# Onr/Council-GAN

Hardware: NVIDIA H100
Metric: training images/sec (gen+dis step) (higher is better)
Workload: dtype tf32

## Files before the change

council_gan_b200/csrc/api.cu:

```cuda
#include "common.cuh"
#include <string.h>

namespace cg {

static thread_local char g_err[512] = "";
std::atomic<uint64_t> g_launches{0};
thread_local int g_tc_mode = 7;
thread_local int g_pdl = 0;

void set_error(const char* fmt, ...) {
    va_list ap;
    va_start(ap, fmt);
    vsnprintf(g_err, sizeof(g_err), fmt, ap);
    va_end(ap);
}

int validate_geom(const cg_conv_geom& g) {
    CG_REQUIRE(g.G >= 1 && (g.x_groups == 1 || g.x_groups == g.G), "conv: x_groups=%d must be 1 or G=%d", g.x_groups, g.G);
    CG_REQUIRE(g.Cin % 4 == 0 && g.Cin > 0, "conv: Cin=%d must be a positive multiple of 4", g.Cin);
    CG_REQUIRE(g.Cout > 0 && g.B > 0 && g.H > 0 && g.W > 0, "conv: empty tensor");
    CG_REQUIRE(g.stride >= 1 && g.KH >= 1 && g.KW >= 1 && g.pad >= 0, "conv: bad kernel geometry");
    int Hin = g.ups ? 2 * g.H : g.H, Win = g.ups ? 2 * g.W : g.W;
    int Ho = (Hin + 2 * g.pad - g.KH) / g.stride + 1, Wo = (Win + 2 * g.pad - g.KW) / g.stride + 1;
    CG_REQUIRE(Ho == g.Ho && Wo == g.Wo, "conv: output size %dx%d inconsistent with geometry (expected %dx%d)", g.Ho, g.Wo, Ho, Wo);
// ... 91 lines not shown
    }
    if (sm_count) *sm_count = prop.multiProcessorCount;
    if (cc_major) *cc_major = prop.major;
    if (cc_minor) *cc_minor = prop.minor;
    return prop.multiProcessorCount;
}

extern "C" int cg_set_tensor_core_mode(int mode) {
    int prev = g_tc_mode;
    g_tc_mode = mode == 1 ? 7 : (mode & 7);
    g_small_bn = ((mode >> 23) & 1) ? 0 : 1;
    g_wgrad_tma = ((mode >> 25) & 1) ? 0 : 1;
    g_pdl = (mode >> 22) & 1;
    g_tc_serial_epilogue = (mode >> 26) & 1;
    g_tc_reg_epilogue = (mode >> 27) & 1;
    return prev;
}

extern "C" uint64_t cg_launch_count(void) { return g_launches.load(); }
extern "C" void cg_tensor_map_cache_stats(uint64_t* hits, uint64_t* misses) { tc_map_cache_stats(hits, misses); }

extern "C" int cg_zero(void* ptr, size_t bytes, void* stream) {
    cudaError_t e = cudaMemsetAsync(ptr, 0, bytes, (cudaStream_t)stream);
    if (e != cudaSuccess) {
        set_error("cg_zero: %s", cudaGetErrorString(e));
        return CG_ERR_CUDA;
    }
    return CG_OK;
}

// ... 146 lines not shown
```

council_gan_b200/csrc/common.cuh:

```cuda
#pragma once
#include <cuda.h>
#include <cuda_runtime.h>
#include <stdint.h>
#include <stdio.h>
#include <stdarg.h>
#include <atomic>
#include "../../include/council_b200.h"

namespace cg {

void set_error(const char* fmt, ...);
extern std::atomic<uint64_t> g_launches;
extern thread_local int g_tc_mode;
extern thread_local int g_small_bn;
extern thread_local int g_wgrad_tma;
extern thread_local int g_tc_serial_epilogue;
extern thread_local int g_tc_reg_epilogue;

constexpr int CG_MAX_DEVICES = 64;
inline int current_device() {
    int dev = 0;
    cudaGetDevice(&dev);
    return dev >= 0 && dev < CG_MAX_DEVICES ? dev : 0;
}
struct PerDeviceOnce {
    std::atomic<bool> done[CG_MAX_DEVICES];
    bool first() { return !done[current_device()].exchange(true); }
    void reset() { done[current_device()].store(false); }
};

inline int check_launch(const char* what) {
    g_launches.fetch_add(1, std::memory_order_relaxed);
// ... 101 lines not shown
```

council_gan_b200/csrc/conv_tc.cu:

```cuda
#include "common.cuh"
#include "tc_ptx.cuh"
#include <cstdlib>
#include <cstdio>
#include <cuda.h>
#include <mutex>
#include <string.h>

namespace cg {

typedef CUresult (*EncodeTiledFn)(CUtensorMap*, CUtensorMapDataType, cuuint32_t, void*, const cuuint64_t*, const cuuint64_t*,
                                  const cuuint32_t*, const cuuint32_t*, CUtensorMapInterleave, CUtensorMapSwizzle,
                                  CUtensorMapL2promotion, CUtensorMapFloatOOBfill);
typedef CUresult (*EncodeIm2colFn)(CUtensorMap*, CUtensorMapDataType, cuuint32_t, void*, const cuuint64_t*, const cuuint64_t*,
                                   const int*, const int*, cuuint32_t, cuuint32_t, const cuuint32_t*, CUtensorMapInterleave,
                                   CUtensorMapSwizzle, CUtensorMapL2promotion, CUtensorMapFloatOOBfill);
typedef CUresult (*ReplaceAddressFn)(CUtensorMap*, void*);
static EncodeTiledFn g_encode_tiled = nullptr;
static ReplaceAddressFn g_replace_address = nullptr;
static EncodeIm2colFn g_encode_im2col = nullptr;
static int g_sm_count_dev[CG_MAX_DEVICES] = {0};
static int sm_count_now() {
    int dev = current_device();
    if (!g_sm_count_dev[dev]) cudaDeviceGetAttribute(&g_sm_count_dev[dev], cudaDevAttrMultiProcessorCount, dev);
    return g_sm_count_dev[dev];
}
thread_local int g_small_bn = 1;
thread_local int g_tc_serial_epilogue = 0;
thread_local int g_tc_reg_epilogue = 0;
static int g_driver_version = 0;
static std::once_flag g_once;

struct MapKey {
    const void* ptr;
    int64_t a, b;
    int32_t v[8];
    bool operator==(const MapKey& o) const { return ptr == o.ptr && a == o.a && b == o.b && memcmp(v, o.v, sizeof(v)) == 0; }
};
struct MapSlot {
    MapKey key;
    CUtensorMap map;
    bool used;
};
constexpr int MAP_SLOTS = 8192;
// ... 41 lines not shown
            g_encode_tiled = (EncodeTiledFn)fn;
        fn = nullptr;
        if (cudaGetDriverEntryPoint("cuTensorMapEncodeIm2col", &fn, cudaEnableDefault, &q) == cudaSuccess && q == cudaDriverEntryPointSuccess)
            g_encode_im2col = (EncodeIm2colFn)fn;
        fn = nullptr;
        if (cudaGetDriverEntryPoint("cuTensorMapReplaceAddress", &fn, cudaEnableDefault, &q) == cudaSuccess && q == cudaDriverEntryPointSuccess)
            g_replace_address = (ReplaceAddressFn)fn;
        cudaDriverGetVersion(&g_driver_version);
    });
}

constexpr int TC_BM = 128;
constexpr int TC_BK = 32;
constexpr int TC_THREADS = 384;
constexpr int TC_MAX_STAGES = 12;
constexpr int TC_MAX_CLASSES = 4;

struct TcClass {
    CUtensorMap amap;
    int w0, h0;
    int out_h0, out_w0;
    int wrow_off;
    int pad_;
};
struct TcParams {
    CUtensorMap bmap;
    TcClass cls[TC_MAX_CLASSES];
    int ncls;
    int G, xg_images;
    int B, P, Q;
// ... 2 lines not shown
    int bk;
    int cps;
    int n_store;
    int out_H, out_W, out_sh, out_sw;
    int w_rows_per_group;
    float* y; const float* bias; const float* addend; const float* mask_src;
    float* stats;
    long stats_gbc;
    int act; float slope;
    int stages;
    int serial_epilogue;
    CUtensorMap ymap, addmap, maskmap;
    int epi_slots, epi_slot_bytes;
};

__device__ __forceinline__ void tc_tile(const TcParams& p, int t, int MT, int NT, int& mt, int& nt, int& c, int& g) {
    if (p.serial_epilogue) {
        mt = t % MT;
        int r = t / MT;
        nt = r % NT;
        r /= NT;
        c = r % p.ncls;
        g = r / p.ncls;
        return;
    }
    c = t % p.ncls;
    int r = t / p.ncls;
    mt = r % MT;
    r /= MT;
    nt = r % NT;
    g = r / NT;
}

__device__ __forceinline__ void tc_half_coords(const TcParams& p, int g, int mt, int h, int& q, int& n) {
    const int pq = p.P * p.Q;
    const int m = mt * TC_BM + 64 * h;
    const int img = m / pq, rem = m - img * pq;
    const int pp = rem / p.Q;
    q = rem - pp * p.Q;
    n = (g * p.B + img) * (p.out_H / p.out_sh) + pp;
}

template <int BK, int BN>
__global__ void __launch_bounds__(TC_THREADS, 1) conv_tc_kernel(const __grid_constant__ TcParams p) {
    pdl_trigger();
    extern __shared__ __align__(1024) uint8_t smem_raw[];
    uint8_t* smem = reinterpret_cast<uint8_t*>((reinterpret_cast<uintptr_t>(smem_raw) + 1023) & ~(uintptr_t)1023);
    const int wg = __shfl_sync(0xffffffffu, threadIdx.x >> 7, 0), tid = threadIdx.x & 127;
    constexpr int a_bytes = TC_BM * BK * 4;
    constexpr int b_bytes = ((BN * BK * 4) + 1023) & ~1023;
    const int stage_bytes = p.cps * (a_bytes + b_bytes);
    constexpr int tx_chunk = a_bytes + BN * BK * 4;
    constexpr bool tma_epi = BK == 32 && BN >= 64;
    const int epi_slots = tma_epi ? p.epi_slots : 0;
    uint8_t* epi = smem + (size_t)p.stages * stage_bytes;
    uint64_t* full_bar = reinterpret_cast<uint64_t*>(epi + (size_t)epi_slots * p.epi_slot_bytes);
    uint64_t* empty_bar = full_bar + p.stages;
    uint64_t* efull_bar = empty_bar + p.stages;
    uint64_t* eempty_bar = efull_bar + epi_slots;

    const int MT = (p.B * p.P * p.Q + TC_BM - 1) / TC_BM;
    const int NT = (p.Cout + BN - 1) / BN;
    const int tiles = p.G * p.ncls * NT * MT;
    const int kchunks = (p.Cin + BK - 1) / BK;
    const int kiters = p.KH * p.KW * kchunks;

    if (threadIdx.x == 0) {
// ... 6 lines not shown
        if (epi_slots) {
            prefetch_tmap(&p.ymap);
            if (p.addend) prefetch_tmap(&p.addmap);
            if (p.mask_src) prefetch_tmap(&p.maskmap);
        }
        for (int s = 0; s < epi_slots; s++) {
            mbar_init(&efull_bar[s], 1);
            mbar_init(&eempty_bar[s], 2);
        }
        fence_barrier_init();
    }
    __syncthreads();
    pdl_wait();

    if (wg == 0) {
        if (tid == 0) {
            int stage = 0;
            uint32_t phase = 0;
            for (int t = blockIdx.x; t < tiles; t += gridDim.x) {
                int mt, nt, c, g;
                tc_tile(p, t, MT, NT, mt, nt, c, g);
                const TcClass& cl = p.cls[c];
                long m0 = (long)mt * TC_BM;
                int img = (int)(m0 / (p.P * p.Q));
                int rem = (int)(m0 - (long)img * p.P * p.Q);
                int pp = rem / p.Q, qq = rem - pp * p.Q;
                int n_coord = g * p.xg_images + img;
                int w_coord = cl.w0 + qq * p.stride;
                int h_coord = cl.h0 + pp * p.stride;
                int wrow = g * p.w_rows_per_group + cl.wrow_off + nt * BN;
                int kh = 0, kw = 0, kc = 0;
                for (int k0 = 0; k0 < kiters; k0 += p.cps) {
                    const int n = kiters - k0 < p.cps ? kiters - k0 : p.cps;
                    mbar_wait(&empty_bar[stage], phase ^ 1);
                    uint8_t* sa = smem + (size_t)stage * stage_bytes;
                    uint8_t* sb = sa + p.cps * a_bytes;
                    mbar_expect_tx(&full_bar[stage], (uint32_t)(n * tx_chunk));
                    for (int j = 0; j < n; j++) {
                        tma_load_im2col_4d(&cl.amap, &full_bar[stage], sa + j * a_bytes, kc * BK, w_coord, h_coord, n_coord, (uint16_t)kw,
                                           (uint16_t)kh);
                        tma_load_2d(&p.bmap, &full_bar[stage], sb + j * b_bytes, (kh * p.KW + kw) * p.Cin + kc * BK, wrow);
                        if (++kc == kchunks) { kc = 0; if (++kw == p.KW) { kw = 0; ++kh; } }
                    }
                    if (++stage == p.stages) { stage = 0; phase ^= 1; }
                }
            }
        } else if (tid == 32 && epi_slots) {
            const uint32_t ebytes = (p.addend ? 2 * 8192 : 0) + (p.mask_src ? 2 * 8192 : 0);
            int es = 0;
            uint32_t ephase = 0;
            for (int t = blockIdx.x; t < tiles; t += gridDim.x) {
                int mt, nt, c, g;
                tc_tile(p, t, MT, NT, mt, nt, c, g);
                const TcClass& cl = p.cls[c];
                int q[2], n[2];
                tc_half_coords(p, g, mt, 0, q[0], n[0]);
                tc_half_coords(p, g, mt, 1, q[1], n[1]);
                for (int sl = 0; sl < BN / 32; sl++) {
                    mbar_wait(&eempty_bar[es], ephase ^ 1);
                    if (ebytes) {
                        mbar_expect_tx(&efull_bar[es], ebytes);
                        uint8_t* dst = epi + (size_t)es * p.epi_slot_bytes;
                        const int c0 = nt * BN + 32 * sl;
                        for (int h = 0; h < 2; h++) {
                            if (p.addend) tma_load_5d(&p.addmap, &efull_bar[es], dst + h * 8192, c0, cl.out_w0, q[h], cl.out_h0, n[h]);
                            if (p.mask_src)
                                tma_load_5d(&p.maskmap, &efull_bar[es], dst + (p.addend ? 16384 : 0) + h * 8192, c0, cl.out_w0, q[h],
                                            cl.out_h0, n[h]);
                        }
                    } else {
                        mbar_arrive(&efull_bar[es]);
                    }
                    if (++es == epi_slots) { es = 0; ephase ^= 1; }
                }
            }
        }
        return;
    }

    const int cw = wg - 1;
    const int warp4 = tid >> 5, lane = tid & 31;
    const int row0 = cw * 64 + warp4 * 16 + (lane >> 2);
    const int cq = 2 * (lane & 3);
    const uint64_t desc0 = BK == 32 ? make_kmajor_sw128_desc(0) : make_kmajor_sw32_desc(0);
    float acc[BN / 2];
    int stage = 0;
    uint32_t phase = 0;
    int es = 0;
    uint32_t ephase = 0;
    for (int t = blockIdx.x; t < tiles; t += gridDim.x) {
        int mt, nt, c, g;
        tc_tile(p, t, MT, NT, mt, nt, c, g);
        const TcClass& cl = p.cls[c];
        int prev = -1;
        for (int k0 = 0; k0 < kiters; k0 += p.cps) {
            const int n = kiters - k0 < p.cps ? kiters - k0 : p.cps;
            mbar_wait(&full_bar[stage], phase);
            const uint32_t sa = smem_u32(smem + (size_t)stage * stage_bytes) + cw * (64 * BK * 4);
            const uint32_t sb = smem_u32(smem + (size_t)stage * stage_bytes) + p.cps * a_bytes;
            wgmma_fence();
            for (int j = 0; j < n; j++) {
                const uint64_t adesc = desc0 | (uint64_t)(((sa + j * a_bytes) & 0x3FFFF) >> 4);
                const uint64_t bdesc = desc0 | (uint64_t)(((sb + j * b_bytes) & 0x3FFFF) >> 4);
#pragma unroll
                for (int kk = 0; kk < BK / 8; kk++)
                    wgmma_tf32<BN>(acc, adesc + (uint64_t)(kk * 2), bdesc + (uint64_t)(kk * 2), (k0 | j | kk) != 0 ? 1 : 0);
            }
// ... 142 lines not shown
                const int j = j0 + jj, col = 8 * j + cq;
#pragma unroll
                for (int h = 0; h < 2; h++) {
                    if (col >= p.n_store || !valid[h]) continue;
                    float2 o = make_float2(acc[4 * j + 2 * h] + 0.f, acc[4 * j + 2 * h + 1] + 0.f);
                    if (p.addend) { o.x += av[jj][h].x; o.y += av[jj][h].y; }
                    if (p.mask_src) { o.x *= mv[jj][h].x > 0.f ? 1.f : p.slope; o.y *= mv[jj][h].y > 0.f ? 1.f : p.slope; }
                    *reinterpret_cast<float2*>(p.y + out_off[h] + col) = o;
                }
            }
        }
    }
    if (epi_slots && tid == 0) bulk_wait<0>();
}


static int encode_weights_map_raw(CUtensorMap* map, const float* w, long rows, long ktot, int bn, int bk) {
    cuuint64_t dims[2] = {(cuuint64_t)ktot, (cuuint64_t)rows};
    cuuint64_t strides[1] = {(cuuint64_t)ktot * 4};
    cuuint32_t box[2] = {(cuuint32_t)bk, (cuuint32_t)bn};
    cuuint32_t estr[2] = {1, 1};
    CUresult r = g_encode_tiled(map, CU_TENSOR_MAP_DATA_TYPE_TFLOAT32, 2, (void*)w, dims, strides, box, estr,
                                CU_TENSOR_MAP_INTERLEAVE_NONE, bk == 32 ? CU_TENSOR_MAP_SWIZZLE_128B : CU_TENSOR_MAP_SWIZZLE_32B,
                                CU_TENSOR_MAP_L2_PROMOTION_L2_256B, CU_TENSOR_MAP_FLOAT_OOB_FILL_NONE);
    if (r != CUDA_SUCCESS) {
        set_error("cuTensorMapEncodeTiled(weights rows=%ld ktot=%ld bn=%d) failed: %d", rows, ktot, bn, (int)r);
        return CG_ERR_CUDA;
    }
    return CG_OK;
}

static int encode_weights_map(CUtensorMap* map, const float* w, long rows, long ktot, int bn, int bk = TC_BK) {
    MapKey k{};
    k.ptr = w; k.a = rows; k.b = ktot; k.v[0] = bn; k.v[1] = bk; k.v[7] = 1;
    return cached_map(map, k, [&](CUtensorMap* m) { return encode_weights_map_raw(m, w, rows, ktot, bn, bk); });
}

static int encode_weights_map_p(TcParams& p, const float* w, long rows, long ktot) {
    return encode_weights_map(&p.bmap, w, rows, ktot, p.bn, p.bk);
}

static int encode_act_map_raw(CUtensorMap* map, const float* x, long N, int H, int W, int C, int lo_w, int lo_h, int up_w, int up_h,
                              int stride, int bk) {
    cuuint64_t dims[4] = {(cuuint64_t)C, (cuuint64_t)W, (cuuint64_t)H, (cuuint64_t)N};
    cuuint64_t strides[3] = {(cuuint64_t)C * 4, (cuuint64_t)W * C * 4, (cuuint64_t)H * W * C * 4};
    int lower[2] = {lo_w, lo_h};
    int upper[2] = {up_w, up_h};
    cuuint32_t estr[4] = {1, (cuuint32_t)stride, (cuuint32_t)stride, 1};
    CUresult r = g_encode_im2col(map, CU_TENSOR_MAP_DATA_TYPE_TFLOAT32, 4, (void*)x, dims, strides, lower, upper, bk, TC_BM, estr,
                                 CU_TENSOR_MAP_INTERLEAVE_NONE, bk == 32 ? CU_TENSOR_MAP_SWIZZLE_128B : CU_TENSOR_MAP_SWIZZLE_32B,
                                 CU_TENSOR_MAP_L2_PROMOTION_L2_128B, CU_TENSOR_MAP_FLOAT_OOB_FILL_NONE);
    if (r != CUDA_SUCCESS) {
        set_error("cuTensorMapEncodeIm2col(N=%ld H=%d W=%d C=%d corners %d,%d / %d,%d stride %d) failed: %d", N, H, W, C, lo_w, lo_h,
                  up_w, up_h, stride, (int)r);
// ... 67 lines not shown
    if ((long)g.B * (g.ups ? g.H * g.W : g.Ho * g.Wo) < TC_BM) return false;
    return true;
}

template <int BK>
static void (*tc_kernel_for(int bn))(TcParams) {
    switch (bn) {
        case 16: return conv_tc_kernel<BK, 16>;
        case 64: return conv_tc_kernel<BK, 64>;
        case 128: return conv_tc_kernel<BK, 128>;
        case 256: return conv_tc_kernel<BK, 256>;
    }
    return nullptr;
}

static int launch_tc(TcParams& p, cudaStream_t st) {
    int a_bytes = TC_BM * p.bk * 4, b_bytes = ((p.bn * p.bk * 4) + 1023) & ~1023;
    int chunk_bytes = a_bytes + b_bytes;
    int kiters = p.KH * p.KW * ((p.Cin + p.bk - 1) / p.bk);
    int cps = p.bn <= 64 ? 2 : 1;
    if (p.bk == 8) cps = 8;
    while (cps > 1 && (cps > kiters || cps * chunk_bytes > 64 * 1024)) cps >>= 1;
    p.cps = cps;
    int stage_bytes = cps * chunk_bytes;
    int stages = (226 * 1024 - 1024 - 2 * TC_MAX_STAGES * 8) / stage_bytes;
    if (stages > TC_MAX_STAGES) stages = TC_MAX_STAGES;
    if (stages > 4 && stage_bytes >= 48 * 1024) stages = 4;
    if (p.n_store == 0) p.n_store = p.bn;
    p.serial_epilogue = g_tc_serial_epilogue;
    p.epi_slots = 0;
    const int nops = (p.addend ? 1 : 0) + (p.mask_src ? 1 : 0);
    const bool aligned = ((uintptr_t)p.y | (uintptr_t)p.addend | (uintptr_t)p.mask_src) % 16 == 0;
    if (g_replace_address && !g_tc_reg_epilogue && !p.serial_epilogue && p.bk == TC_BK && p.bn >= 64 && p.n_store == p.bn && (long)p.P * p.Q % TC_BM == 0 &&
        (p.Q % 64 == 0 || 64 % p.Q == 0) && p.out_H % p.out_sh == 0 && p.out_W % p.out_sw == 0 && p.Cout % 4 == 0 && aligned) {
        const int slot_bytes = (nops ? nops : 1) * 16384;
        auto slots_beside = [&](int st) { return (int)((227L * 1024 - 1024 - (long)st * stage_bytes - 2 * st * 8) / (slot_bytes + 16)); };
        while (slots_beside(stages) < 2 && stages > 4) stages--;
        const int e = slots_beside(stages);
        if (e >= 2) {
            p.epi_slots = e < 4 ? e : 4;
            p.epi_slot_bytes = slot_bytes;
            const long ni = (long)p.G * p.B;
            const int qbox = p.Q < 64 ? p.Q : 64;
            if (int rc = encode_out_map(&p.ymap, p.y, ni, p.out_H, p.out_W, p.Cout, p.out_sh, p.out_sw, qbox)) return rc;
            if (p.addend)
                if (int rc = encode_out_map(&p.addmap, p.addend, ni, p.out_H, p.out_W, p.Cout, p.out_sh, p.out_sw, qbox)) return rc;
            if (p.mask_src)
                if (int rc = encode_out_map(&p.maskmap, p.mask_src, ni, p.out_H, p.out_W, p.Cout, p.out_sh, p.out_sw, qbox)) return rc;
        }
    }
    p.stages = stages;
    size_t smem = (size_t)stages * stage_bytes + 1024  + 2 * stages * 8 + (size_t)p.epi_slots * (p.epi_slot_bytes + 16);
    void (*kern)(TcParams) = p.bk == 32 ? tc_kernel_for<32>(p.bn) : tc_kernel_for<8>(p.bn);
    if (!kern) {
        set_error("conv_tc: no kernel for N tile %d / K chunk %d", p.bn, p.bk);
        return CG_ERR_ARG;
    }
    static PerDeviceOnce attr_set;
    if (attr_set.first()) {
        for (int bn : {16, 64, 128, 256}) {
            cudaError_t e = cudaFuncSetAttribute(tc_kernel_for<32>(bn), cudaFuncAttributeMaxDynamicSharedMemorySize, 227 * 1024);
            if (e == cudaSuccess) e = cudaFuncSetAttribute(tc_kernel_for<8>(bn), cudaFuncAttributeMaxDynamicSharedMemorySize, 227 * 1024);
            if (e != cudaSuccess) {
                attr_set.reset();
                set_error("cudaFuncSetAttribute(conv_tc_kernel): %s", cudaGetErrorString(e));
                return CG_ERR_CUDA;
            }
        }
    }
    int MT = cdiv((long)p.B * p.P * p.Q, TC_BM);
    long tiles = (long)p.G * p.ncls * ((p.Cout + p.bn - 1) / p.bn) * MT;
    const long slots = sm_count_now();
    int grid = (int)(tiles < slots ? tiles : slots);
    launch_k(kern, grid, TC_THREADS, smem, st, p);
    return check_launch("conv_tc_kernel");
}


__global__ void ups_weight_transform_kernel(const float* __restrict__ w, float* __restrict__ wc, long total, int Cout, int Cin) {
    pdl_trigger();
    pdl_wait();
    long i = (long)blockIdx.x * blockDim.x + threadIdx.x;
    if (i >= total) return;
    int ci = (int)(i % Cin);
    long t = i / Cin;
    int ss = (int)(t % 2); t /= 2;
    int r = (int)(t % 2); t /= 2;
    int co = (int)(t % Cout); t /= Cout;
    int cls = (int)(t % 4);
    int g = (int)(t / 4);
// ... 30 lines not shown
    p.bk = pick_bk(g.Cin);
    long nimg = (long)(g.x_groups == 1 ? 1 : g.G) * g.B;
    p.G = g.G; p.xg_images = g.x_groups == 1 ? 0 : g.B;
    p.B = g.B; p.Cin = g.Cin; p.Cout = g.Cout;
    p.y = y; p.bias = bias; p.addend = nullptr; p.mask_src = nullptr; p.act = act; p.slope = slope;
    if (g.ups) {
        size_t need = tc_fwd_ws(g);
        if (need > ws_bytes) {
            set_error("conv_fwd(tc, upsample classes): workspace %zu < %zu bytes", ws_bytes, need);
            return CG_ERR_WORKSPACE;
        }
        float* wc = (float*)ws;
        long total = (long)g.G * 4 * g.Cout * 4 * g.Cin;
        launch_k(ups_weight_transform_kernel, cdiv(total, 256), 256, 0, st, w, wc, total, g.Cout, g.Cin);
        if (int rc = check_launch("ups_weight_transform")) return rc;
        if (int rc = encode_weights_map_p(p, wc, (long)g.G * 4 * g.Cout, 4L * g.Cin)) return rc;
        for (int c = 0; c < 4; c++) {
            int a = c >> 1, b = c & 1;
            int lo_h = a == 0 ? -1 : 0, lo_w = b == 0 ? -1 : 0;
            int up_h = a == 0 ? -1 : 0, up_w = b == 0 ? -1 : 0;
            if (int rc = encode_act_map(&p.cls[c].amap, x, nimg, g.H, g.W, g.Cin, lo_w, lo_h, up_w, up_h, 1, p.bk)) return rc;
            p.cls[c].w0 = lo_w; p.cls[c].h0 = lo_h; p.cls[c].out_h0 = a; p.cls[c].out_w0 = b; p.cls[c].wrow_off = c * g.Cout;
        }
        p.ncls = 4;
        p.P = g.H; p.Q = g.W; p.KH = 2; p.KW = 2; p.stride = 1;
        p.out_H = g.Ho; p.out_W = g.Wo; p.out_sh = 2; p.out_sw = 2;
        p.w_rows_per_group = 4 * g.Cout;
        return launch_tc(p, st);
    }
    long ktot = (long)g.KH * g.KW * g.Cin;
    if (int rc = encode_weights_map_p(p, w, (long)g.G * g.Cout, ktot)) return rc;
    if (int rc = encode_act_map(&p.cls[0].amap, x, nimg, g.H, g.W, g.Cin, -g.pad, -g.pad, g.pad - (g.KW - 1), g.pad - (g.KH - 1), g.stride,
                                p.bk))
        return rc;
    p.cls[0].w0 = -g.pad; p.cls[0].h0 = -g.pad; p.cls[0].out_h0 = 0; p.cls[0].out_w0 = 0; p.cls[0].wrow_off = 0;
    p.ncls = 1;
    p.P = g.Ho; p.Q = g.Wo;
    p.KH = g.KH; p.KW = g.KW; p.stride = g.stride;
    p.out_H = g.Ho; p.out_W = g.Wo; p.out_sh = 1; p.out_sw = 1;
    p.w_rows_per_group = g.Cout;
    return launch_tc(p, st);
}

__global__ void __launch_bounds__(256) dgrad_weight_transform_kernel(const float* __restrict__ w, float* __restrict__ wt, int Cout, int Cin,
                                                                     int CinP, int KH, int KW, int s) {
    pdl_trigger();
    pdl_wait();
    __shared__ float tile[32][33];
    const int TH = KH / s, TW = KW / s;
    const int cit = (CinP + 31) / 32;
    const int co0 = (blockIdx.x / cit) * 32, ci0 = (blockIdx.x % cit) * 32;
    int t = blockIdx.y;
    const int ss = t % TW; t /= TW;
    const int r = t % TH; t /= TH;
    const int cls = t;
    const int g = blockIdx.z;
// ... 46 lines not shown
    float* wt = (float*)ws;
    const int CinP = g.Cin <= 16 ? 16 : g.Cin;
    size_t wt_bytes = ((size_t)g.G * g.Cout * g.KH * g.KW * CinP * sizeof(float) + 1023) & ~(size_t)1023;
    float* d_seen = g.ups ? (float*)((uint8_t*)ws + wt_bytes) : dx;
    long total = (long)g.G * g.Cout * g.KH * g.KW * CinP;
    (void)total;
    launch_k(dgrad_weight_transform_kernel, dim3(cdiv(g.Cout, 32) * cdiv(CinP, 32), g.KH * g.KW, g.G), dim3(32, 8), 0, st, w, wt, g.Cout, g.Cin, CinP,
                                                                                                                  g.KH, g.KW, s);
    if (int rc = check_launch("dgrad_weight_transform")) return rc;

    TcParams p{};
    p.bn = pick_bn(g.Cin);
    if (p.bn > 64) p.bn = fill_bn(p.bn, (long)g.B * ((g.ups ? 2 * g.H : g.H) / g.stride) * ((g.ups ? 2 * g.W : g.W) / g.stride), g.G * g.stride * g.stride, g.Cin);
    p.n_store = p.bn == 16 ? g.Cin : p.bn;
    p.bk = pick_bk(g.Cout);
    long ktot = (long)TH * TW * g.Cout;
    if (int rc = encode_weights_map_p(p, wt, (long)g.G * ncls * CinP, ktot)) return rc;
    for (int c = 0; c < ncls; c++) {
        int ph = c / s, pw = c - ph * s;
        int ihf = ((ph - g.pad) % s + s) % s, iwf = ((pw - g.pad) % s + s) % s;
        int padl_h = (TH - 1) - (ihf + g.pad - ph) / s, padl_w = (TW - 1) - (iwf + g.pad - pw) / s;
        int Hc = Hin / s, Wc = Win / s;
        int up_h = Hc - g.Ho - padl_h, up_w = Wc - g.Wo - padl_w;
        if (int rc = encode_act_map(&p.cls[c].amap, dy, (long)g.G * g.B, g.Ho, g.Wo, g.Cout, -padl_w, -padl_h, up_w, up_h, 1, p.bk)) return rc;
        p.cls[c].w0 = -padl_w; p.cls[c].h0 = -padl_h;
        p.cls[c].out_h0 = ihf; p.cls[c].out_w0 = iwf;
        p.cls[c].wrow_off = c * CinP;
    }
    p.ncls = ncls;
    p.G = g.G; p.xg_images = g.B;
    p.B = g.B; p.P = Hin / s; p.Q = Win / s;
    p.Cin = g.Cout; p.Cout = g.Cin; p.KH = TH; p.KW = TW; p.stride = 1;
    p.out_H = Hin; p.out_W = Win; p.out_sh = s; p.out_sw = s;
    p.w_rows_per_group = ncls * CinP;
    p.y = d_seen; p.bias = nullptr;
    p.addend = g.ups ? nullptr : addend; p.mask_src = g.ups ? nullptr : mask_src;
    p.act = CG_ACT_NONE; p.slope = mask_slope;
    if (int rc = launch_tc(p, st)) return rc;
    if (g.ups) return pool2x2_sum(d_seen, dx, addend, mask_src, mask_slope, (long)g.G * g.B, g.H, g.W, g.Cin, st);
    return CG_OK;
}


constexpr int WG_BK = 32;

struct WgParams {
    const float* x; const float* dy; float* out;
    int G, xg_images, B, H, W, Ho, Wo, Cin, Cout, KH, KW, stride, pad;
    long Mpix, chunk;
    int ci_tiles;
};

__device__ __forceinline__ float f4_at(const float4& v, int j) { return j == 0 ? v.x : j == 1 ? v.y : j == 2 ? v.z : v.w; }
// ... 525 lines not shown
```

council_gan_b200/csrc/tc_ptx.cuh:

```cuda
#pragma once
#include <cuda.h>
#include <cuda_runtime.h>
#include <stdint.h>

namespace cg {

__device__ __forceinline__ uint32_t smem_u32(const void* p) { return (uint32_t)__cvta_generic_to_shared(p); }

__device__ __forceinline__ void mbar_init(uint64_t* bar, uint32_t count) {
    asm volatile("mbarrier.init.shared::cta.b64 [%0], %1;" ::"r"(smem_u32(bar)), "r"(count));
}
__device__ __forceinline__ void mbar_expect_tx(uint64_t* bar, uint32_t bytes) {
    asm volatile("mbarrier.arrive.expect_tx.shared::cta.b64 _, [%0], %1;" ::"r"(smem_u32(bar)), "r"(bytes) : "memory");
}
__device__ __forceinline__ void mbar_arrive(uint64_t* bar) {
    asm volatile("mbarrier.arrive.shared::cta.b64 _, [%0];" ::"r"(smem_u32(bar)) : "memory");
}
__device__ __forceinline__ void mbar_wait(uint64_t* bar, uint32_t parity) {
    uint32_t done;
    const uint32_t addr = smem_u32(bar);
    do {
        asm volatile(
            "{\n"
            ".reg .pred p;\n"
// ... 33 lines not shown
        "cp.async.bulk.tensor.5d.shared::cluster.global.mbarrier::complete_tx::bytes [%0], [%1, {%3, %4, %5, %6, %7}], [%2];" ::"r"(smem_u32(dst)),
        "l"(map), "r"(smem_u32(bar)), "r"(c0), "r"(c1), "r"(c2), "r"(c3), "r"(c4)
        : "memory");
}
__device__ __forceinline__ void tma_store_5d(const CUtensorMap* map, const void* src, int c0, int c1, int c2, int c3, int c4) {
    asm volatile("cp.async.bulk.tensor.5d.global.shared::cta.tile.bulk_group [%0, {%2, %3, %4, %5, %6}], [%1];" ::"l"(map),
                 "r"(smem_u32(src)), "r"(c0), "r"(c1), "r"(c2), "r"(c3), "r"(c4)
                 : "memory");
}
__device__ __forceinline__ void bulk_commit() { asm volatile("cp.async.bulk.commit_group;" ::: "memory"); }
template <int N>
__device__ __forceinline__ void bulk_wait_read() { asm volatile("cp.async.bulk.wait_group.read %0;" ::"n"(N) : "memory"); }
template <int N>
__device__ __forceinline__ void bulk_wait() { asm volatile("cp.async.bulk.wait_group %0;" ::"n"(N) : "memory"); }
__device__ __forceinline__ void named_bar_sync(int id, int count) { asm volatile("bar.sync %0, %1;" ::"r"(id), "r"(count) : "memory"); }
__device__ __forceinline__ void prefetch_tmap(const CUtensorMap* map) {
    asm volatile("prefetch.tensormap [%0];" ::"l"(map) : "memory");
}

__device__ __forceinline__ uint64_t make_kmajor_sw128_desc(uint32_t smem_addr) {
    uint64_t d = 0;
    d |= (uint64_t)((smem_addr & 0x3FFFF) >> 4);
    d |= (uint64_t)1 << 16;
    d |= (uint64_t)(1024 >> 4) << 32;
    d |= (uint64_t)1 << 62;
    return d;
}
__device__ __forceinline__ uint64_t make_kmajor_sw32_desc(uint32_t smem_addr) {
    uint64_t d = 0;
    d |= (uint64_t)((smem_addr & 0x3FFFF) >> 4);
// ... 86 lines not shown
```

Before: 47.78.

## Add ping-pong consumer warpgroup conv kernel with register reallocation

Adds a ping-pong variant of the TMA/WGMMA implicit-GEMM conv kernel. The two consumer warpgroups take alternate tiles, and turn-taking mbarriers let one warpgroup's epilogue overlap the other's MMA main loop. The producer warpgroup gives up registers via setmaxnreg so the consumers can grow theirs. The N tile is forced to 128 with an N-inner tile order. The path is used by default when the smem epilogue applies and there are enough tiles; the cost is a narrower tile and extra turn synchronisation.

```diff
diff --git a/council_gan_b200/csrc/api.cu b/council_gan_b200/csrc/api.cu
--- a/council_gan_b200/csrc/api.cu
+++ b/council_gan_b200/csrc/api.cu
@@ -129,6 +129,7 @@
     g_pdl = (mode >> 22) & 1;
     g_tc_serial_epilogue = (mode >> 26) & 1;
     g_tc_reg_epilogue = (mode >> 27) & 1;
+    g_tc_coop = (mode >> 28) & 1;
     return prev;
 }
 
diff --git a/council_gan_b200/csrc/common.cuh b/council_gan_b200/csrc/common.cuh
--- a/council_gan_b200/csrc/common.cuh
+++ b/council_gan_b200/csrc/common.cuh
@@ -16,6 +16,7 @@
 extern thread_local int g_wgrad_tma;
 extern thread_local int g_tc_serial_epilogue;
 extern thread_local int g_tc_reg_epilogue;
+extern thread_local int g_tc_coop;
 
 constexpr int CG_MAX_DEVICES = 64;
 inline int current_device() {
diff --git a/council_gan_b200/csrc/conv_tc.cu b/council_gan_b200/csrc/conv_tc.cu
--- a/council_gan_b200/csrc/conv_tc.cu
+++ b/council_gan_b200/csrc/conv_tc.cu
@@ -27,6 +27,7 @@
 thread_local int g_small_bn = 1;
 thread_local int g_tc_serial_epilogue = 0;
 thread_local int g_tc_reg_epilogue = 0;
+thread_local int g_tc_coop = 0;
 static int g_driver_version = 0;
 static std::once_flag g_once;
 
@@ -98,6 +99,7 @@
 constexpr int TC_BK = 32;
 constexpr int TC_THREADS = 384;
 constexpr int TC_MAX_STAGES = 12;
+constexpr int TC_PP_BN = 128;
 constexpr int TC_MAX_CLASSES = 4;
 
 struct TcClass {
@@ -130,7 +132,17 @@
     int epi_slots, epi_slot_bytes;
 };
 
+template <bool N_INNER>
 __device__ __forceinline__ void tc_tile(const TcParams& p, int t, int MT, int NT, int& mt, int& nt, int& c, int& g) {
+    if constexpr (N_INNER) {
+        c = t % p.ncls;
+        int r = t / p.ncls;
+        nt = r % NT;
+        r /= NT;
+        mt = r % MT;
+        g = r / MT;
+        return;
+    }
     if (p.serial_epilogue) {
         mt = t % MT;
         int r = t / MT;
@@ -155,6 +167,77 @@
     const int pp = rem / p.Q;
     q = rem - pp * p.Q;
     n = (g * p.B + img) * (p.out_H / p.out_sh) + pp;
+}
+
+template <int BK, int BN, bool N_INNER>
+__device__ __forceinline__ void tc_produce(const TcParams& p, uint8_t* smem, uint64_t* full_bar, uint64_t* empty_bar, int tiles, int MT,
+                                           int NT, int kchunks, int kiters, int stage_bytes) {
+    constexpr int a_bytes = TC_BM * BK * 4;
+    constexpr int b_bytes = ((BN * BK * 4) + 1023) & ~1023;
+    constexpr int tx_chunk = a_bytes + BN * BK * 4;
+    int stage = 0;
+    uint32_t phase = 0;
+    for (int t = blockIdx.x; t < tiles; t += gridDim.x) {
+        int mt, nt, c, g;
+        tc_tile<N_INNER>(p, t, MT, NT, mt, nt, c, g);
+        const TcClass& cl = p.cls[c];
+        long m0 = (long)mt * TC_BM;
+        int img = (int)(m0 / (p.P * p.Q));
+        int rem = (int)(m0 - (long)img * p.P * p.Q);
+        int pp = rem / p.Q, qq = rem - pp * p.Q;
+        int n_coord = g * p.xg_images + img;
+        int w_coord = cl.w0 + qq * p.stride;
+        int h_coord = cl.h0 + pp * p.stride;
+        int wrow = g * p.w_rows_per_group + cl.wrow_off + nt * BN;
+        int kh = 0, kw = 0, kc = 0;
+        for (int k0 = 0; k0 < kiters; k0 += p.cps) {
+            const int n = kiters - k0 < p.cps ? kiters - k0 : p.cps;
+            mbar_wait(&empty_bar[stage], phase ^ 1);
+            uint8_t* sa = smem + (size_t)stage * stage_bytes;
+            uint8_t* sb = sa + p.cps * a_bytes;
+            mbar_expect_tx(&full_bar[stage], (uint32_t)(n * tx_chunk));
+            for (int j = 0; j < n; j++) {
+                tma_load_im2col_4d(&cl.amap, &full_bar[stage], sa + j * a_bytes, kc * BK, w_coord, h_coord, n_coord, (uint16_t)kw,
+                                   (uint16_t)kh);
+                tma_load_2d(&p.bmap, &full_bar[stage], sb + j * b_bytes, (kh * p.KW + kw) * p.Cin + kc * BK, wrow);
+                if (++kc == kchunks) { kc = 0; if (++kw == p.KW) { kw = 0; ++kh; } }
+            }
+            if (++stage == p.stages) { stage = 0; phase ^= 1; }
+        }
+    }
+}
+
+template <int BN, bool N_INNER>
+__device__ __forceinline__ void tc_produce_epi(const TcParams& p, uint8_t* epi, uint64_t* efull_bar, uint64_t* eempty_bar, int tiles, int MT,
+                                               int NT, int epi_slots) {
+    const uint32_t ebytes = (p.addend ? 2 * 8192 : 0) + (p.mask_src ? 2 * 8192 : 0);
+    int es = 0;
+    uint32_t ephase = 0;
+    for (int t = blockIdx.x; t < tiles; t += gridDim.x) {
+        int mt, nt, c, g;
+        tc_tile<N_INNER>(p, t, MT, NT, mt, nt, c, g);
+        const TcClass& cl = p.cls[c];
+        int q[2], n[2];
+        tc_half_coords(p, g, mt, 0, q[0], n[0]);
+        tc_half_coords(p, g, mt, 1, q[1], n[1]);
+        for (int sl = 0; sl < BN / 32; sl++) {
+            mbar_wait(&eempty_bar[es], ephase ^ 1);
+            if (ebytes) {
+                mbar_expect_tx(&efull_bar[es], ebytes);
+                uint8_t* dst = epi + (size_t)es * p.epi_slot_bytes;
+                const int c0 = nt * BN + 32 * sl;
+                for (int h = 0; h < 2; h++) {
+                    if (p.addend) tma_load_5d(&p.addmap, &efull_bar[es], dst + h * 8192, c0, cl.out_w0, q[h], cl.out_h0, n[h]);
+                    if (p.mask_src)
+                        tma_load_5d(&p.maskmap, &efull_bar[es], dst + (p.addend ? 16384 : 0) + h * 8192, c0, cl.out_w0, q[h],
+                                    cl.out_h0, n[h]);
+                }
+            } else {
+                mbar_arrive(&efull_bar[es]);
+            }
+            if (++es == epi_slots) { es = 0; ephase ^= 1; }
+        }
+    }
 }
 
 template <int BK, int BN>
@@ -166,7 +249,6 @@
     constexpr int a_bytes = TC_BM * BK * 4;
     constexpr int b_bytes = ((BN * BK * 4) + 1023) & ~1023;
     const int stage_bytes = p.cps * (a_bytes + b_bytes);
-    constexpr int tx_chunk = a_bytes + BN * BK * 4;
     constexpr bool tma_epi = BK == 32 && BN >= 64;
     const int epi_slots = tma_epi ? p.epi_slots : 0;
     uint8_t* epi = smem + (size_t)p.stages * stage_bytes;
@@ -203,67 +285,8 @@
     pdl_wait();
 
     if (wg == 0) {
-        if (tid == 0) {
-            int stage = 0;
-            uint32_t phase = 0;
-            for (int t = blockIdx.x; t < tiles; t += gridDim.x) {
-                int mt, nt, c, g;
-                tc_tile(p, t, MT, NT, mt, nt, c, g);
-                const TcClass& cl = p.cls[c];
-                long m0 = (long)mt * TC_BM;
-                int img = (int)(m0 / (p.P * p.Q));
-                int rem = (int)(m0 - (long)img * p.P * p.Q);
-                int pp = rem / p.Q, qq = rem - pp * p.Q;
-                int n_coord = g * p.xg_images + img;
-                int w_coord = cl.w0 + qq * p.stride;
-                int h_coord = cl.h0 + pp * p.stride;
-                int wrow = g * p.w_rows_per_group + cl.wrow_off + nt * BN;
-                int kh = 0, kw = 0, kc = 0;
-                for (int k0 = 0; k0 < kiters; k0 += p.cps) {
-                    const int n = kiters - k0 < p.cps ? kiters - k0 : p.cps;
-                    mbar_wait(&empty_bar[stage], phase ^ 1);
-                    uint8_t* sa = smem + (size_t)stage * stage_bytes;
-                    uint8_t* sb = sa + p.cps * a_bytes;
-                    mbar_expect_tx(&full_bar[stage], (uint32_t)(n * tx_chunk));
-                    for (int j = 0; j < n; j++) {
-                        tma_load_im2col_4d(&cl.amap, &full_bar[stage], sa + j * a_bytes, kc * BK, w_coord, h_coord, n_coord, (uint16_t)kw,
-                                           (uint16_t)kh);
-                        tma_load_2d(&p.bmap, &full_bar[stage], sb + j * b_bytes, (kh * p.KW + kw) * p.Cin + kc * BK, wrow);
-                        if (++kc == kchunks) { kc = 0; if (++kw == p.KW) { kw = 0; ++kh; } }
-                    }
-                    if (++stage == p.stages) { stage = 0; phase ^= 1; }
-                }
-            }
-        } else if (tid == 32 && epi_slots) {
-            const uint32_t ebytes = (p.addend ? 2 * 8192 : 0) + (p.mask_src ? 2 * 8192 : 0);
-            int es = 0;
-            uint32_t ephase = 0;
-            for (int t = blockIdx.x; t < tiles; t += gridDim.x) {
-                int mt, nt, c, g;
-                tc_tile(p, t, MT, NT, mt, nt, c, g);
-                const TcClass& cl = p.cls[c];
-                int q[2], n[2];
-                tc_half_coords(p, g, mt, 0, q[0], n[0]);
-                tc_half_coords(p, g, mt, 1, q[1], n[1]);
-                for (int sl = 0; sl < BN / 32; sl++) {
-                    mbar_wait(&eempty_bar[es], ephase ^ 1);
-                    if (ebytes) {
-                        mbar_expect_tx(&efull_bar[es], ebytes);
-                        uint8_t* dst = epi + (size_t)es * p.epi_slot_bytes;
-                        const int c0 = nt * BN + 32 * sl;
-                        for (int h = 0; h < 2; h++) {
-                            if (p.addend) tma_load_5d(&p.addmap, &efull_bar[es], dst + h * 8192, c0, cl.out_w0, q[h], cl.out_h0, n[h]);
-                            if (p.mask_src)
-                                tma_load_5d(&p.maskmap, &efull_bar[es], dst + (p.addend ? 16384 : 0) + h * 8192, c0, cl.out_w0, q[h],
-                                            cl.out_h0, n[h]);
-                        }
-                    } else {
-                        mbar_arrive(&efull_bar[es]);
-                    }
-                    if (++es == epi_slots) { es = 0; ephase ^= 1; }
-                }
-            }
-        }
+        if (tid == 0) tc_produce<BK, BN, false>(p, smem, full_bar, empty_bar, tiles, MT, NT, kchunks, kiters, stage_bytes);
+        else if (tid == 32 && epi_slots) tc_produce_epi<BN, false>(p, epi, efull_bar, eempty_bar, tiles, MT, NT, epi_slots);
         return;
     }
 
@@ -279,7 +302,7 @@
     uint32_t ephase = 0;
     for (int t = blockIdx.x; t < tiles; t += gridDim.x) {
         int mt, nt, c, g;
-        tc_tile(p, t, MT, NT, mt, nt, c, g);
+        tc_tile<false>(p, t, MT, NT, mt, nt, c, g);
         const TcClass& cl = p.cls[c];
         int prev = -1;
         for (int k0 = 0; k0 < kiters; k0 += p.cps) {
@@ -452,6 +475,204 @@
     if (epi_slots && tid == 0) bulk_wait<0>();
 }
 
+template <int BN>
+__global__ void __launch_bounds__(TC_THREADS, 1) conv_tc_pp_kernel(const __grid_constant__ TcParams p) {
+    constexpr int BK = TC_BK;
+    pdl_trigger();
+    extern __shared__ __align__(1024) uint8_t smem_raw[];
+    uint8_t* smem = reinterpret_cast<uint8_t*>((reinterpret_cast<uintptr_t>(smem_raw) + 1023) & ~(uintptr_t)1023);
+    const int wg = __shfl_sync(0xffffffffu, threadIdx.x >> 7, 0), tid = threadIdx.x & 127;
+    constexpr int a_bytes = TC_BM * BK * 4;
+    constexpr int b_bytes = BN * BK * 4;
+    constexpr int stage_bytes = a_bytes + b_bytes;
+    const int epi_slots = p.epi_slots;
+    uint8_t* epi = smem + (size_t)p.stages * stage_bytes;
+    uint64_t* full_bar = reinterpret_cast<uint64_t*>(epi + (size_t)epi_slots * p.epi_slot_bytes);
+    uint64_t* empty_bar = full_bar + p.stages;
+    uint64_t* efull_bar = empty_bar + p.stages;
+    uint64_t* eempty_bar = efull_bar + epi_slots;
+    uint64_t* mma_turn = eempty_bar + epi_slots;
+    uint64_t* epi_turn = mma_turn + 2;
+
+    const int MT = (p.B * p.P * p.Q + TC_BM - 1) / TC_BM;
+    const int NT = (p.Cout + BN - 1) / BN;
+    const int tiles = p.G * p.ncls * NT * MT;
+    const int kchunks = (p.Cin + BK - 1) / BK;
+    const int kiters = p.KH * p.KW * kchunks;
+
+    if (threadIdx.x == 0) {
+        prefetch_tmap(&p.bmap);
+        for (int c = 0; c < p.ncls; c++) prefetch_tmap(&p.cls[c].amap);
+        prefetch_tmap(&p.ymap);
+        if (p.addend) prefetch_tmap(&p.addmap);
+        if (p.mask_src) prefetch_tmap(&p.maskmap);
+        for (int s = 0; s < p.stages; s++) {
+            mbar_init(&full_bar[s], 1);
+            mbar_init(&empty_bar[s], 1);
+        }
+        for (int s = 0; s < epi_slots; s++) {
+            mbar_init(&efull_bar[s], 1);
+            mbar_init(&eempty_bar[s], 1);
+        }
+        for (int w = 0; w < 2; w++) {
+            mbar_init(&mma_turn[w], 1);
+            mbar_init(&epi_turn[w], 1);
+        }
+        fence_barrier_init();
+    }
+    __syncthreads();
+    pdl_wait();
+
+    if (wg == 0) {
+        setmaxnreg_dec<40>();
+        if (tid == 0) tc_produce<BK, BN, true>(p, smem, full_bar, empty_bar, tiles, MT, NT, kchunks, kiters, stage_bytes);
+        else if (tid == 32) tc_produce_epi<BN, true>(p, epi, efull_bar, eempty_bar, tiles, MT, NT, epi_slots);
+        return;
+    }
+    setmaxnreg_inc<232>();
+
+    const int cw = wg - 1;
+    const int warp4 = tid >> 5, lane = tid & 31;
+    const int cq = 2 * (lane & 3);
+    const int r0 = warp4 * 16 + (lane >> 2);
+    const uint64_t desc0 = make_kmajor_sw128_desc(0);
+    constexpr int slices = BN / 32;
+    float acc[2][BN / 2];
+    int stage = 0, es = 0;
+    uint32_t phase = 0, ephase = 0, mma_par = 0, epi_par = 0;
+    int i = 0;
+    for (int t = blockIdx.x; t < tiles; t += gridDim.x, i++) {
+        if ((i & 1) != cw) {
+            stage += kiters;
+            phase ^= (stage / p.stages) & 1;
+            stage %= p.stages;
+            es += slices;
+            ephase ^= (es / epi_slots) & 1;
+            es %= epi_slots;
+            continue;
+        }
+        int mt, nt, c, g;
+        tc_tile<true>(p, t, MT, NT, mt, nt, c, g);
+        const TcClass& cl = p.cls[c];
+        if (i > 0) {
+            mbar_wait(&mma_turn[cw], mma_par);
+            mma_par ^= 1;
+        }
+        int prev = -1;
+        for (int k = 0; k < kiters; k++) {
+            mbar_wait(&full_bar[stage], phase);
+            const uint32_t sa = smem_u32(smem + (size_t)stage * stage_bytes);
+            const uint64_t adesc = desc0 | (uint64_t)((sa & 0x3FFFF) >> 4);
+            const uint64_t bdesc = desc0 | (uint64_t)(((sa + a_bytes) & 0x3FFFF) >> 4);
+            wgmma_fence();
+#pragma unroll
+            for (int kk = 0; kk < BK / 8; kk++) {
+#pragma unroll
+                for (int h = 0; h < 2; h++)
+                    wgmma_tf32<BN>(acc[h], adesc + (uint64_t)(h * (a_bytes / 2 >> 4) + kk * 2), bdesc + (uint64_t)(kk * 2),
+                                   (k | kk) != 0 ? 1 : 0);
+            }
+            wgmma_commit();
+            wgmma_wait<1>();
+            if (prev >= 0 && tid == 0) mbar_arrive(&empty_bar[prev]);
+            prev = stage;
+            if (++stage == p.stages) { stage = 0; phase ^= 1; }
+        }
+        if (tid == 0) mbar_arrive(&mma_turn[cw ^ 1]);
+        wgmma_wait<0>();
+        wgmma_reg_fence(acc[0], BN / 2);
+        wgmma_reg_fence(acc[1], BN / 2);
+        if (tid == 0) mbar_arrive(&empty_bar[prev]);
+
+        if (p.stats) {
+            const int pq = p.P * p.Q;
+            const int tiles_per_img = pq / TC_BM;
+            const int img = (mt * TC_BM) / pq;
+            const int chunk = ((c * tiles_per_img + (mt - img * tiles_per_img)) << 3) + warp4;
+            const bool b2 = lane & 4, b3 = lane & 8;
+#pragma unroll
+            for (int h = 0; h < 2; h++) {
+                float* st = p.stats + ((long)(chunk + 4 * h) * p.stats_gbc + (long)(g * p.B + img) * p.Cout + nt * BN + cq) * 2 + (b3 ? 2 : 0) +
+                            (b2 ? 1 : 0);
+                const float* a = acc[h];
+#pragma unroll
+                for (int j = 0; j < BN / 8; j++) {
+                    const float s0 = a[4 * j] + a[4 * j + 2], s1 = a[4 * j + 1] + a[4 * j + 3];
+                    const float q0 = a[4 * j] * a[4 * j] + a[4 * j + 2] * a[4 * j + 2];
+                    const float q1 = a[4 * j + 1] * a[4 * j + 1] + a[4 * j + 3] * a[4 * j + 3];
+                    const float k0 = b2 ? q0 : s0, k1 = b2 ? q1 : s1;
+                    const float x0 = k0 + __shfl_xor_sync(0xffffffffu, b2 ? s0 : q0, 4), x1 = k1 + __shfl_xor_sync(0xffffffffu, b2 ? s1 : q1, 4);
+                    float v = (b3 ? x1 : x0) + __shfl_xor_sync(0xffffffffu, b3 ? x0 : x1, 8);
+                    v += __shfl_xor_sync(0xffffffffu, v, 16);
+                    if (lane < 16) st[16 * j] = v;
+                }
+            }
+        }
+
+        if (i > 0) {
+            mbar_wait(&epi_turn[cw], epi_par);
+            epi_par ^= 1;
+        }
+        int q[2], n[2];
+        tc_half_coords(p, g, mt, 0, q[0], n[0]);
+        tc_half_coords(p, g, mt, 1, q[1], n[1]);
+#pragma unroll
+        for (int sl = 0; sl < slices; sl++) {
+            float2 bv[4];
+#pragma unroll
+            for (int jj = 0; jj < 4; jj++)
+                bv[jj] = p.bias ? __ldg(reinterpret_cast<const float2*>(p.bias + (long)g * p.Cout + nt * BN + 32 * sl + 8 * jj + cq))
+                                : make_float2(0.f, 0.f);
+            mbar_wait(&efull_bar[es], ephase);
+            uint8_t* slot = epi + (size_t)es * p.epi_slot_bytes;
+#pragma unroll
+            for (int hm = 0; hm < 2; hm++) {
+                uint8_t* half = slot + hm * 8192;
+                const uint8_t* msk = half + (p.addend ? 16384 : 0);
+#pragma unroll
+                for (int jj = 0; jj < 4; jj++) {
+                    const int j = 4 * sl + jj;
+#pragma unroll
+                    for (int h = 0; h < 2; h++) {
+                        const int r = r0 + 8 * h;
+                        const int off = r * 128 + (((2 * jj + (cq >> 2)) ^ (r & 7)) << 4) + (cq & 3) * 4;
+                        float2 o = make_float2(acc[hm][4 * j + 2 * h] + bv[jj].x, acc[hm][4 * j + 2 * h + 1] + bv[jj].y);
+                        if (p.addend) {
+                            const float2 a = *reinterpret_cast<const float2*>(half + off);
+                            o.x += a.x; o.y += a.y;
+                        }
+                        if (p.mask_src) {
+                            const float2 a = *reinterpret_cast<const float2*>(msk + off);
+                            o.x *= a.x > 0.f ? 1.f : p.slope; o.y *= a.y > 0.f ? 1.f : p.slope;
+                        } else if (p.act != CG_ACT_NONE) {
+                            o.x = apply_act(o.x, p.act, p.slope); o.y = apply_act(o.y, p.act, p.slope);
+                        }
+                        *reinterpret_cast<float2*>(half + off) = o;
+                    }
+                }
+            }
+            fence_proxy_async();
+            named_bar_sync(1 + cw, 128);
+            if (tid == 0) {
+                tma_store_5d(&p.ymap, slot, nt * BN + 32 * sl, cl.out_w0, q[0], cl.out_h0, n[0]);
+                tma_store_5d(&p.ymap, slot + 8192, nt * BN + 32 * sl, cl.out_w0, q[1], cl.out_h0, n[1]);
+                bulk_commit();
+                if (sl > 0) {
+                    bulk_wait_read<1>();
+                    mbar_arrive(&eempty_bar[es == 0 ? epi_slots - 1 : es - 1]);
+                }
+                if (sl == slices - 1) {
+                    bulk_wait_read<0>();
+                    mbar_arrive(&eempty_bar[es]);
+                    mbar_arrive(&epi_turn[cw ^ 1]);
+                }
+            }
+            if (++es == epi_slots) { es = 0; ephase ^= 1; }
+        }
+    }
+    if (tid == 0) bulk_wait<0>();
+}
+
 
 static int encode_weights_map_raw(CUtensorMap* map, const float* w, long rows, long ktot, int bn, int bk) {
     cuuint64_t dims[2] = {(cuuint64_t)ktot, (cuuint64_t)rows};
@@ -472,10 +693,6 @@
     MapKey k{};
     k.ptr = w; k.a = rows; k.b = ktot; k.v[0] = bn; k.v[1] = bk; k.v[7] = 1;
     return cached_map(map, k, [&](CUtensorMap* m) { return encode_weights_map_raw(m, w, rows, ktot, bn, bk); });
-}
-
-static int encode_weights_map_p(TcParams& p, const float* w, long rows, long ktot) {
-    return encode_weights_map(&p.bmap, w, rows, ktot, p.bn, p.bk);
 }
 
 static int encode_act_map_raw(CUtensorMap* map, const float* x, long N, int H, int W, int C, int lo_w, int lo_h, int up_w, int up_h,
@@ -573,7 +790,19 @@
     return nullptr;
 }
 
-static int launch_tc(TcParams& p, cudaStream_t st) {
+static int launch_tc(TcParams& p, const float* w, long w_rows, long w_ktot, cudaStream_t st) {
+    if (p.n_store == 0) p.n_store = p.bn;
+    p.serial_epilogue = g_tc_serial_epilogue;
+    const int nops = (p.addend ? 1 : 0) + (p.mask_src ? 1 : 0);
+    const bool aligned = ((uintptr_t)p.y | (uintptr_t)p.addend | (uintptr_t)p.mask_src) % 16 == 0;
+    const bool smem_epi = g_replace_address && !g_tc_reg_epilogue && !p.serial_epilogue && p.bk == TC_BK && p.bn >= 64 && p.n_store == p.bn &&
+                          (long)p.P * p.Q % TC_BM == 0 && (p.Q % 64 == 0 || 64 % p.Q == 0) && p.out_H % p.out_sh == 0 &&
+                          p.out_W % p.out_sw == 0 && p.Cout % 4 == 0 && aligned;
+    const long MT = cdiv((long)p.B * p.P * p.Q, TC_BM);
+    const bool pp = smem_epi && !g_tc_coop && (p.bn == 128 || p.bn == 256) &&
+                    (long)p.G * p.ncls * (p.Cout / TC_PP_BN) * MT >= 2L * sm_count_now();
+    if (pp) p.bn = p.n_store = TC_PP_BN;
+    if (int rc = encode_weights_map(&p.bmap, w, w_rows, w_ktot, p.bn, p.bk)) return rc;
     int a_bytes = TC_BM * p.bk * 4, b_bytes = ((p.bn * p.bk * 4) + 1023) & ~1023;
     int chunk_bytes = a_bytes + b_bytes;
     int kiters = p.KH * p.KW * ((p.Cin + p.bk - 1) / p.bk);
@@ -585,15 +814,13 @@
     int stages = (226 * 1024 - 1024 - 2 * TC_MAX_STAGES * 8) / stage_bytes;
     if (stages > TC_MAX_STAGES) stages = TC_MAX_STAGES;
     if (stages > 4 && stage_bytes >= 48 * 1024) stages = 4;
-    if (p.n_store == 0) p.n_store = p.bn;
-    p.serial_epilogue = g_tc_serial_epilogue;
+    const int turn_bytes = pp ? 4 * 8 : 0;
     p.epi_slots = 0;
-    const int nops = (p.addend ? 1 : 0) + (p.mask_src ? 1 : 0);
-    const bool aligned = ((uintptr_t)p.y | (uintptr_t)p.addend | (uintptr_t)p.mask_src) % 16 == 0;
-    if (g_replace_address && !g_tc_reg_epilogue && !p.serial_epilogue && p.bk == TC_BK && p.bn >= 64 && p.n_store == p.bn && (long)p.P * p.Q % TC_BM == 0 &&
-        (p.Q % 64 == 0 || 64 % p.Q == 0) && p.out_H % p.out_sh == 0 && p.out_W % p.out_sw == 0 && p.Cout % 4 == 0 && aligned) {
+    if (smem_epi) {
         const int slot_bytes = (nops ? nops : 1) * 16384;
-        auto slots_beside = [&](int st) { return (int)((227L * 1024 - 1024 - (long)st * stage_bytes - 2 * st * 8) / (slot_bytes + 16)); };
+        auto slots_beside = [&](int st) {
+            return (int)((227L * 1024 - 1024 - (long)st * stage_bytes - 2 * st * 8 - turn_bytes) / (slot_bytes + 16));
+        };
         while (slots_beside(stages) < 2 && stages > 4) stages--;
         const int e = slots_beside(stages);
         if (e >= 2) {
@@ -609,30 +836,32 @@
         }
     }
     p.stages = stages;
-    size_t smem = (size_t)stages * stage_bytes + 1024  + 2 * stages * 8 + (size_t)p.epi_slots * (p.epi_slot_bytes + 16);
-    void (*kern)(TcParams) = p.bk == 32 ? tc_kernel_for<32>(p.bn) : tc_kernel_for<8>(p.bn);
+    const bool pp_run = pp && p.epi_slots;
+    size_t smem = (size_t)stages * stage_bytes + 1024  + 2 * stages * 8 + (size_t)p.epi_slots * (p.epi_slot_bytes + 16) +
+                  (pp_run ? turn_bytes : 0);
+    void (*kern)(TcParams) = pp_run ? conv_tc_pp_kernel<TC_PP_BN> : p.bk == 32 ? tc_kernel_for<32>(p.bn) : tc_kernel_for<8>(p.bn);
     if (!kern) {
         set_error("conv_tc: no kernel for N tile %d / K chunk %d", p.bn, p.bk);
         return CG_ERR_ARG;
     }
     static PerDeviceOnce attr_set;
     if (attr_set.first()) {
+        cudaError_t e = cudaFuncSetAttribute(conv_tc_pp_kernel<TC_PP_BN>, cudaFuncAttributeMaxDynamicSharedMemorySize, 227 * 1024);
         for (int bn : {16, 64, 128, 256}) {
-            cudaError_t e = cudaFuncSetAttribute(tc_kernel_for<32>(bn), cudaFuncAttributeMaxDynamicSharedMemorySize, 227 * 1024);
+            if (e == cudaSuccess) e = cudaFuncSetAttribute(tc_kernel_for<32>(bn), cudaFuncAttributeMaxDynamicSharedMemorySize, 227 * 1024);
             if (e == cudaSuccess) e = cudaFuncSetAttribute(tc_kernel_for<8>(bn), cudaFuncAttributeMaxDynamicSharedMemorySize, 227 * 1024);
-            if (e != cudaSuccess) {
-                attr_set.reset();
-                set_error("cudaFuncSetAttribute(conv_tc_kernel): %s", cudaGetErrorString(e));
-                return CG_ERR_CUDA;
-            }
-        }
-    }
-    int MT = cdiv((long)p.B * p.P * p.Q, TC_BM);
+        }
+        if (e != cudaSuccess) {
+            attr_set.reset();
+            set_error("cudaFuncSetAttribute(conv_tc_kernel): %s", cudaGetErrorString(e));
+            return CG_ERR_CUDA;
+        }
+    }
     long tiles = (long)p.G * p.ncls * ((p.Cout + p.bn - 1) / p.bn) * MT;
     const long slots = sm_count_now();
     int grid = (int)(tiles < slots ? tiles : slots);
     launch_k(kern, grid, TC_THREADS, smem, st, p);
-    return check_launch("conv_tc_kernel");
+    return check_launch(pp_run ? "conv_tc_pp_kernel" : "conv_tc_kernel");
 }
 
 
@@ -693,7 +922,6 @@
         long total = (long)g.G * 4 * g.Cout * 4 * g.Cin;
         launch_k(ups_weight_transform_kernel, cdiv(total, 256), 256, 0, st, w, wc, total, g.Cout, g.Cin);
         if (int rc = check_launch("ups_weight_transform")) return rc;
-        if (int rc = encode_weights_map_p(p, wc, (long)g.G * 4 * g.Cout, 4L * g.Cin)) return rc;
         for (int c = 0; c < 4; c++) {
             int a = c >> 1, b = c & 1;
             int lo_h = a == 0 ? -1 : 0, lo_w = b == 0 ? -1 : 0;
@@ -705,10 +933,8 @@
         p.P = g.H; p.Q = g.W; p.KH = 2; p.KW = 2; p.stride = 1;
         p.out_H = g.Ho; p.out_W = g.Wo; p.out_sh = 2; p.out_sw = 2;
         p.w_rows_per_group = 4 * g.Cout;
-        return launch_tc(p, st);
-    }
-    long ktot = (long)g.KH * g.KW * g.Cin;
-    if (int rc = encode_weights_map_p(p, w, (long)g.G * g.Cout, ktot)) return rc;
+        return launch_tc(p, wc, (long)g.G * 4 * g.Cout, 4L * g.Cin, st);
+    }
     if (int rc = encode_act_map(&p.cls[0].amap, x, nimg, g.H, g.W, g.Cin, -g.pad, -g.pad, g.pad - (g.KW - 1), g.pad - (g.KH - 1), g.stride,
                                 p.bk))
         return rc;
@@ -718,7 +944,7 @@
     p.KH = g.KH; p.KW = g.KW; p.stride = g.stride;
     p.out_H = g.Ho; p.out_W = g.Wo; p.out_sh = 1; p.out_sw = 1;
     p.w_rows_per_group = g.Cout;
-    return launch_tc(p, st);
+    return launch_tc(p, w, (long)g.G * g.Cout, (long)g.KH * g.KW * g.Cin, st);
 }
 
 __global__ void __launch_bounds__(256) dgrad_weight_transform_kernel(const float* __restrict__ w, float* __restrict__ wt, int Cout, int Cin,
@@ -795,8 +1021,6 @@
     if (p.bn > 64) p.bn = fill_bn(p.bn, (long)g.B * ((g.ups ? 2 * g.H : g.H) / g.stride) * ((g.ups ? 2 * g.W : g.W) / g.stride), g.G * g.stride * g.stride, g.Cin);
     p.n_store = p.bn == 16 ? g.Cin : p.bn;
     p.bk = pick_bk(g.Cout);
-    long ktot = (long)TH * TW * g.Cout;
-    if (int rc = encode_weights_map_p(p, wt, (long)g.G * ncls * CinP, ktot)) return rc;
     for (int c = 0; c < ncls; c++) {
         int ph = c / s, pw = c - ph * s;
         int ihf = ((ph - g.pad) % s + s) % s, iwf = ((pw - g.pad) % s + s) % s;
@@ -817,7 +1041,7 @@
     p.y = d_seen; p.bias = nullptr;
     p.addend = g.ups ? nullptr : addend; p.mask_src = g.ups ? nullptr : mask_src;
     p.act = CG_ACT_NONE; p.slope = mask_slope;
-    if (int rc = launch_tc(p, st)) return rc;
+    if (int rc = launch_tc(p, wt, (long)g.G * ncls * CinP, (long)TH * TW * g.Cout, st)) return rc;
     if (g.ups) return pool2x2_sum(d_seen, dx, addend, mask_src, mask_slope, (long)g.G * g.B, g.H, g.W, g.Cin, st);
     return CG_OK;
 }
diff --git a/council_gan_b200/csrc/tc_ptx.cuh b/council_gan_b200/csrc/tc_ptx.cuh
--- a/council_gan_b200/csrc/tc_ptx.cuh
+++ b/council_gan_b200/csrc/tc_ptx.cuh
@@ -71,6 +71,10 @@
 template <int N>
 __device__ __forceinline__ void bulk_wait() { asm volatile("cp.async.bulk.wait_group %0;" ::"n"(N) : "memory"); }
 __device__ __forceinline__ void named_bar_sync(int id, int count) { asm volatile("bar.sync %0, %1;" ::"r"(id), "r"(count) : "memory"); }
+template <int N>
+__device__ __forceinline__ void setmaxnreg_dec() { asm volatile("setmaxnreg.dec.sync.aligned.u32 %0;" ::"n"(N)); }
+template <int N>
+__device__ __forceinline__ void setmaxnreg_inc() { asm volatile("setmaxnreg.inc.sync.aligned.u32 %0;" ::"n"(N)); }
 __device__ __forceinline__ void prefetch_tmap(const CUtensorMap* map) {
     asm volatile("prefetch.tensormap [%0];" ::"l"(map) : "memory");
 }
```

New measurement: 49.98 (median of 6 runs). 4.6% higher.
